# mnadareski/ZPAQSharp

Hardware: AMD Instinct MI355X
Metric: decompress MB/s (bit-exact) on 1 GiB multi-block stream (higher is better)
Workload: dtype u32; 1 GPU; BASELINE configs[1]: 256 x 4 MiB independent blocks per GPU, model l1 (1 component(s)), plaintext generator T; zpaq_model=l1, blocks_per_gpu=256, block_bytes=4194304, plaintext=T, parallelism=blocks x1, kernel_kind=2, blocks_in_flight=256

## Files before the change

zpaqsharp_amd/csrc/zh_cm.hip:

```cpp
#include <hip/hip_runtime.h>
#include <stddef.h>
#include <stdint.h>

#include "zh_core.h"
#include "zh_dev.h"
#include "zh_cm_fast.h"
#include "zh_model.h"

using namespace zhcore;
using namespace zhdev;

#pragma clang diagnostic ignored "-Wint-to-pointer-cast"

namespace {

constexpr uint32_t kNoWin = 0xFFFFFFFFu;
constexpr uint32_t kRing = 16;
enum : uint32_t { kMsgByte = 0, kMsgLeave = 2 };
enum : uint32_t { kCmdEnter = 1, kCmdExit = 3 };
constexpr uint32_t kSpinSection = 1u << 27;
constexpr uint64_t kSpinIdle = 1ull << 33;
#define ZH_E_HELPER (-24)

struct alignas(64) CmTabs {
  int16_t sh[16384];
  uint16_t sq[4096];
  int32_t dt[1024];
};
template <uint32_t NW>
struct alignas(64) CmBlkT {
  static constexpr uint32_t kNW = NW;
  uint32_t winB[NW][256];
  uint32_t winA[NW][16];
  uint16_t p16B[NW][256];
  uint16_t p16A[NW][16];
  alignas(64) uint32_t ring[kRing];
  uint32_t dummy[64];
  uint32_t aux[kRing][2];
  uint32_t tags[64];
  uint4 wsink[64];
  alignas(8) uint32_t mreq;
  uint32_t mold, mdone, mcfg;
  uint32_t t0, b_seq;
  uint32_t cmd_seq, cmd_code, cmd_ack;
  uint32_t limit, ob_word, ob_room;
  uint64_t table, ob_base, ob_cap, ob_len, ob_stored;
  uint32_t table_bytes;
  uint32_t pr[256];
  Vm pz;
  Sink sink;
};
template <uint32_t NW, uint32_t NP>
struct alignas(64) CmLdsT {
  CmTabs T;
  CmBlkT<NW> B[NP];
};
static_assert(sizeof(CmLdsT<64, 1>) <= 163840 && sizeof(CmLdsT<32, 2>) <= 163840, "LDS budget");
static_assert(offsetof(CmBlkT<64>, mold) == offsetof(CmBlkT<64>, mreq) + 4 && offsetof(CmBlkT<64>, mdone) == offsetof(CmBlkT<64>, mreq) + 8 && offsetof(CmBlkT<64>, mreq) % 8 == 0, "swap mailbox layout");

__device__ __forceinline__ uint32_t lds_ld(const uint32_t *p) {
  return __hip_atomic_load(p, __ATOMIC_RELAXED, __HIP_MEMORY_SCOPE_WORKGROUP);
}
__device__ __forceinline__ void lds_st(uint32_t *p, uint32_t v) {
  __hip_atomic_store(p, v, __ATOMIC_RELAXED, __HIP_MEMORY_SCOPE_WORKGROUP);
}
__device__ __forceinline__ void lds_put0(const uint32_t *where, uint32_t val) {
  const uint32_t addr = (uint32_t)(uintptr_t)where;
  asm volatile("s_mov_b64 exec, 1\n\tds_write_b32 %0, %1\n\ts_mov_b64 exec, -1" ::"v"(addr), "v"(val) : "memory");
}
__device__ __forceinline__ void lds_order() { asm volatile("" ::: "memory"); }
typedef __attribute__((address_space(3))) uint16_t *lds_u16_p;
typedef __attribute__((address_space(3))) uint32_t *lds_u32_p;
typedef __attribute__((address_space(3))) const uint64_t *lds_u64_p;
__device__ __forceinline__ uint32_t lds_u16(uint32_t off) { return *(lds_u16_p)off; }
__device__ __forceinline__ uint64_t lds_u64(uint32_t off) { return *(lds_u64_p)off; }
__device__ __forceinline__ uint32_t lds_off(const void *p) { return (uint32_t)(uintptr_t)p; }
__device__ __forceinline__ uint32_t p16b_pos(uint32_t q, uint32_t P) { return ((q & 3) << 6) | (P << 2) | (q >> 2); }
__device__ __forceinline__ uint32_t ring_tag(uint32_t u) { return u & 127u; }
static_assert(kRing == 16, "ring_tag");
__device__ __forceinline__ void wave_sync() { __builtin_amdgcn_fence(__ATOMIC_SEQ_CST, "workgroup"); }

__device__ __forceinline__ uint32_t p16_of(const CmTabs &T, uint32_t cm) {
  const uint32_t xv = cm >> 17;
  const int st = xv >= 16384 ? (int)T.sh[xv - 16384] : -(int)T.sh[16383 - xv];
  return (uint32_t)T.sq[st + 2048] * 2 + 1;
}

template <class BLK>
__device__ __forceinline__ void win_store(const BLK &S, uint32_t slot, uint32_t *table, uint32_t w, uint32_t lane) {
  uint4 *g = reinterpret_cast<uint4 *>(table + (uint64_t)w * 512);
// ... 143 lines not shown
    const uint32_t n = (r >> 23) & 255u;
    if (n == done) {
      const uint32_t c = uni(cfg_now);
      if (c == ~0u) break;
      if (++idle > 64) __builtin_amdgcn_s_sleep(2);
      if (idle > kSpinIdle) break;
      continue;
    }
    idle = 0;
    if (PROF) { asm volatile("s_memtime %0\n\ts_waitcnt lgkmcnt(0)" : "=s"(t_req)::"memory"); }
    const uint32_t c = uni(cfg_now);
    if (UNLIKELY(c != cfg)) {
      cfg = c;
      __builtin_amdgcn_fence(__ATOMIC_ACQUIRE, "workgroup");
      trs = __builtin_amdgcn_make_buffer_rsrc((void *)(L.arena + uni64(S.table)), 0, (int)uni(S.table_bytes), 0x00020000);
    }
    const uint32_t sl = r & 63u;
    const uint32_t neww = (r >> 22) & 1u ? uni(S.aux[0][0]) : (r >> 6) & 0xFFFFu;
    const uint32_t oldw = uni((uint32_t)(rq >> 32));
    const uint32_t aB = l_cB + sl * 1024u, aA = l_cA + sl * l_mA, aP = l_cP + sl * l_mP;
    const uint32_t so_new = neww * 2048u;
    const v4u nb = __builtin_amdgcn_raw_buffer_load_b128(trs, g_offB, so_new, 0);
    const v4u na = __builtin_amdgcn_raw_buffer_load_b128(trs, g_offA, so_new, 0);
    const v4u np = __builtin_amdgcn_raw_buffer_load_b128(trs, g_offP, so_new, 0);
    if (oldw != kNoWin) {
      const v4u vb = *(lds_v4_p)aB, va = *(lds_v4_p)aA, vp = *(lds_v4_p)aP;
      const uint32_t so_old = oldw * 2048u;
      __builtin_amdgcn_raw_buffer_store_b128(vb, trs, g_offB, so_old, 0);
      __builtin_amdgcn_raw_buffer_store_b128(va, trs, g_offA, so_old, 0);
      __builtin_amdgcn_raw_buffer_store_b128(vp, trs, g_offP, so_old, 0);
    }
    if (PROF) { asm volatile("s_memtime %0\n\ts_waitcnt lgkmcnt(0)" : "=s"(t_out)::"memory"); asm volatile("s_waitcnt vmcnt(3)" ::: "memory");
                asm volatile("s_memtime %0\n\ts_waitcnt lgkmcnt(0)" : "=s"(t_back)::"memory"); }
    *(lds_v4_p)aB = nb;
    *(lds_v4_p)aA = na;
    *(lds_v4_p)aP = np;
    lds_order();
    lds_put0(&S.mdone, n);
    done = n;
    if (PROF) { asm volatile("s_waitcnt lgkmcnt(0)\n\ts_memtime %0\n\ts_waitcnt lgkmcnt(0)" : "=s"(t_done)::"memory");
                c_a += t_out - t_req; c_b += t_back - t_out; c_c += t_done - t_back; ++n_sw; }
  }
  if (PROF && lane == 0 && L.debug) {
    atomicAdd((unsigned long long *)&L.debug[13], (unsigned long long)c_a);
    atomicAdd((unsigned long long *)&L.debug[14], (unsigned long long)c_b);
    atomicAdd((unsigned long long *)&L.debug[15], (unsigned long long)c_c);
    atomicAdd((unsigned long long *)&L.debug[9], (unsigned long long)n_sw);
  }
}

template <bool PROF, uint32_t NW, uint32_t NP>
__device__ __forceinline__ void decode_cm_body(const ZhLaunch &L, CmLdsT<NW, NP> &SS) {
  uint64_t prof[16] = {0, 0, 0, 0, 0, 0, 0, 0, 0, 0, 0, 0, 0, 0, 0, 0};
  uint64_t tprev = 0, t_exit = 0, t_pub = 0;
  bool was_miss = false;
  const uint32_t lane = threadIdx.x & 63, wid = threadIdx.x >> 6, pair = NP > 1 ? wid % NP : 0u, wave = NP > 1 ? wid / NP : wid;
  CmTabs &T = SS.T;
  CmBlkT<NW> &S = SS.B[pair];

  {
    const uint4 *s0 = reinterpret_cast<const uint4 *>(L.tables->stretch + 16384);
    uint4 *d0 = reinterpret_cast<uint4 *>(T.sh);
    for (uint32_t i = threadIdx.x; i < sizeof(T.sh) / 16; i += 192 * NP) d0[i] = s0[i];
    const uint4 *s1 = reinterpret_cast<const uint4 *>(L.tables->squash);
    uint4 *d1 = reinterpret_cast<uint4 *>(T.sq);
    for (uint32_t i = threadIdx.x; i < sizeof(T.sq) / 16; i += 192 * NP) d1[i] = s1[i];
    const uint4 *s2 = reinterpret_cast<const uint4 *>(L.tables->dt);
    uint4 *d2 = reinterpret_cast<uint4 *>(T.dt);
    for (uint32_t i = threadIdx.x; i < sizeof(T.dt) / 16; i += 192 * NP) d2[i] = s2[i];
    if (wave == 0 && lane == 0) { S.cmd_seq = 0; S.cmd_code = 0; S.cmd_ack = 0; S.t0 = 0; S.b_seq = 0; S.mreq = 0; S.mold = 0; S.mdone = 0; S.mcfg = 0; }
  }
  __syncthreads();
  if (wave == 1) { helper_wave<PROF>(L, T, S, lane); return; }
  if (wave == 2) { swap_wave<PROF>(L, S, lane); return; }
  uint32_t n_miss = 0, sec_cfg = 0;
  uint32_t cmd_seq = 0;

  const uint32_t l15 = lane & 15;
  const uint32_t lgrp = lane >> 4;
  const uint32_t ltt = 31 - __clz((int)(l15 | 1));
  const uint32_t lsh_vis = 4 - ltt, lsh_y = 3 - ltt;
  const uint32_t p_la = lds_off(&S.p16A[0][0]) + l15 * 2, p_lb = lds_off(&S.p16B[0][0]) + lgrp * 128 + l15 * 8;
  const uint32_t ring_addr = lds_off(&S.ring[0]), bseq_addr = lds_off(&S.b_seq), mreq_addr = lds_off(&S.mreq);
  const uint32_t dummy_addr = lds_off(&S.dummy[lane]), ring_step = lane == 0 ? 63u : 0u;

  uint8_t *slot_mem = L.arena + (uint64_t)(blockIdx.x * NP + pair) * L.arena_stride;

  for (;;) {
    uint32_t bi = 0;
    if (lane == 0) bi = atomicAdd(L.queue, 1u);
    bi = uni((uint32_t)__shfl((int)bi, 0));
    if (bi >= L.n_blocks) break;

    const ZhBlockDesc *bdp = &L.blocks[bi];
    const uint32_t model_i = uni(bdp->model);
    const uint32_t first_seg = uni(bdp->first_seg), n_seg = uni(bdp->n_seg);
    const uint64_t b_out_off = uni64(bdp->out_off), b_out_cap = uni64(bdp->out_cap);
    const ZhModel *M = &L.models[model_i];
    const ZhComp *cp = &M->comp[0];
    const uint32_t cm_mask = uni(cp->cm_mask);
    const uint32_t limit = (uint32_t)uni(cp->arg[1]) * 4;
    const uint64_t cm_off = uni64(cp->cm_off), cm_bytes = uni64(cp->cm_bytes);
    const uint32_t win_bfe = 9u | ((uint32_t)__builtin_popcount(cm_mask) - 9u) << 16;
    const uint32_t hshift = (uni(M->kind) >> 16) & 255;
    uint32_t *table = reinterpret_cast<uint32_t *>(slot_mem + cm_off);

    {
      const uint4 v = make_uint4(0x80000000u, 0x80000000u, 0x80000000u, 0x80000000u);
      uint4 *q = reinterpret_cast<uint4 *>(table);
      for (uint64_t i = lane; i < cm_bytes / 16; i += 64) q[i] = v;
      const uint32_t pv = p16_of(T, 0x80000000u), pp = pv | pv << 16;
      const uint4 ppat = make_uint4(pp, pp, pp, pp);
      const uint64_t nwin = cm_bytes / 2048;
      for (uint64_t i = lane; i < nwin * 34; i += 64) {
        const uint64_t w = i / 34, k = i % 34;
        q[w * 128 + (k < 32 ? 8 + k : 4 + (k - 32))] = ppat;
      }
      const uint64_t h_off = uni64(M->h_off), tail = uni64(M->arena_bytes) - h_off;
      uint4 *z = reinterpret_cast<uint4 *>(slot_mem + h_off);
      for (uint64_t i = lane; i < tail / 16; i += 64) z[i] = make_uint4(0, 0, 0, 0);
      for (uint32_t i = lane; i < 256; i += 64) S.pr[i] = 0;
    }
    wave_sync();

    uint32_t tag = kNoWin;
    uint32_t stale = 0;
    uint32_t lastuse = lane < NW ? 0u : ~0u;
    uint32_t thr = 1;
    uint32_t t = 0;
    uint32_t h0 = 0;

    int pp_state = 0, pp_hsize = 0;
    uint32_t pp_len = 0;
    Vm &pz = S.pz;
    pz.a = pz.b = pz.c = pz.d = pz.f = 0;
    pz.prog = nullptr; pz.len = 0;
    pz.m = slot_mem + uni64(M->pm_off); pz.mmask = (uint32_t)((1ull << uni(M->pm)) - 1);
    pz.h = reinterpret_cast<uint32_t *>(slot_mem + uni64(M->ph_off)); pz.hmask = (uint32_t)((1ull << uni(M->ph)) - 1);
    pz.r = S.pr;
    uint8_t *pzbuf = slot_mem + uni64(M->pz_off) + ZH_CODE_PAD;

    Dec d;
    d.low = 1; d.high = 0xFFFFFFFFu; d.curr = 0;

    OutBuf ob;
    ob.base = L.out + b_out_off; ob.cap = b_out_cap; ob.len = 0; ob.stored = 0; ob.word = 0; ob.park = 0;
    out_room(ob);
    Sink &sink = S.sink;
    sink.out = ob.base; sink.cap = ob.cap; sink.len = 0;

    wave_sync();
    InBuf in;
    in.stream = L.in; in.total = L.in_total; in.cbase = 0; in.k = 0; in.avail = 0; in.cur = 0;

    int failed = 0;
    for (uint32_t s = 0; s < n_seg; ++s) {
      const uint32_t si = first_seg + s;
      const uint64_t produced0 = pp_state == 5 ? uni64(sink.len) : ob.len;
      int status = 0;
      if (failed) {
        if (lane == 0) {
          ZhSegResult res;
          res.status = ZH_E_SKIPPED; res.pp_state = (uint32_t)pp_state; res.out_off = b_out_off + produced0; res.out_len = 0;
          res.in_used = 0;
          L.results[si] = res;
        }
// ... 68 lines not shown
          for (int i = 0; i < 4; ++i) {
            const uint32_t ps = rdlane(psel, lb + j2);
            ZH_DEC_STEP(d, ps, j2, bad, rn);
            if (UNLIKELY(rn)) { if (dec_renorm(d, in, lane) && !err) err = bad ? (uint32_t)-ZH_E_CORRUPT : (uint32_t)-ZH_E_EOF; }
          }
          if (UNLIKELY(err | bad)) { status = err ? -(int)err : ZH_E_CORRUPT; return -2; }
          ZH_STAMP(4);
          const uint32_t n2 = j2 & 15;
          c = (int)(n1 << 4 | n2);

          {
            const bool isb = lgrp == (ga & 3);
            const bool isa = lgrp == ((ga & 3) ^ 1);
            const uint32_t cmsel = kb == 0 ? cmb[0] : kb == 1 ? cmb[1] : kb == 2 ? cmb[2] : cmb[3];
            const uint32_t cm = isb ? cmsel : cma;
            const uint32_t nib = isb ? n2 : n1;
            const bool vis = (isa || isb) && l15 != 0 && l15 == ((16 | nib) >> lsh_vis);
            const uint32_t yy = (nib >> lsh_y) & 1;
            const uint32_t cnt = cm & 0x3ff;
            const int e = (int)(yy * 32767) - (int)(cm >> 17);
            const uint32_t nv = cm + (((uint32_t)e * (uint32_t)T.dt[cnt]) & 0xFFFFFC00u) + (cnt < limit);
            if (vis) { if (isb) wb[ib0 + 64 * kb] = nv; else wa[l15] = nv; }
          }
          ZH_STAMP(5);
          h0 = (uint32_t)c << hshift;
        }
        return (int)uni((uint32_t)c);
      };

      for (;;) {
        if (LIKELY(pp_state == 1)) {
          S.tags[lane] = stale;
          stale = 0;
          if (lane < kRing) S.ring[lane] = ((ring_tag(t) + 64) & 127) << 25;
          out_flush(ob, lane);
          if (lane == 0) {
            S.table = (uint64_t)(reinterpret_cast<uint8_t *>(table) - L.arena); S.limit = limit;
            S.table_bytes = (uint32_t)(cm_bytes > 0xFFFFF000ull ? 0xFFFFF000ull : cm_bytes);
            S.mcfg = ++sec_cfg;
            S.ob_base = (uint64_t)(ob.base - L.out); S.ob_cap = ob.cap; S.ob_len = ob.len; S.ob_stored = ob.stored;
            S.ob_word = ob.word; S.ob_room = ob.room;
            S.t0 = t; S.b_seq = t; S.cmd_code = kCmdEnter;
          }
          __builtin_amdgcn_fence(__ATOMIC_RELEASE, "workgroup");
          ++cmd_seq;
          lds_st(&S.cmd_seq, cmd_seq);
          bool helper_ok = true;
          {
            uint32_t sp = 0;
            while (lds_ld(&S.cmd_ack) != cmd_seq) { if (++sp > kSpinSection) { helper_ok = false; break; } }
            __builtin_amdgcn_fence(__ATOMIC_ACQUIRE, "workgroup");
          }
          if (!helper_ok) { status = ZH_E_HELPER; break; }
          uint32_t b_done = t;
          auto publish = [&](uint32_t m0) __attribute__((always_inline)) {
            lds_order();
            lds_put0(&S.ring[t & (kRing - 1)], ring_tag(t) << 25 | m0);
            ++t;
          };
          auto wait_done = [&](uint32_t upto) __attribute__((always_inline)) -> bool {
            uint32_t sp = 0;
            while ((int32_t)(b_done - upto) < 0) {
              b_done = uni(lds_ld(&S.b_seq));
              if (++sp > kSpinSection) return false;
            }
            lds_order();
            return true;
          };
          enum : uint32_t { kEvEos = 1, kEvCorrupt, kEvEof, kEvHelper };
          uint32_t ev = 0;
          uint32_t tq;
          for (;;) {
            {
              if (in.avail - in.k < 49 && in.avail == 256) in_seek(in, in_pos(in), lane);
              uint32_t code;
              d.low = uni(d.low); d.high = uni(d.high); d.curr = uni(d.curr); in.k = uni(in.k); in.avail = uni(in.avail);
              t = uni(t); h0 = uni(h0); b_done = uni(b_done); n_miss = uni(n_miss); thr = uni(thr);
              uint64_t f0 = 0, f1 = 0;
              const uint32_t t_in = t;
              if (PROF) { asm volatile("s_memtime %0\n\ts_waitcnt lgkmcnt(0)" : "=s"(f0)::"memory"); }
              if (LIKELY(d.curr - d.low <= d.high - d.low && t < 0x3e000000u)) {
                const uint32_t klim = uni(in.avail >= 48 ? in.avail - 48 : 0u);
                uint32_t vr = lane == 0 ? ring_addr + (t & (kRing - 1)) * 4u : dummy_addr;
                if (PROF) {
                  uint32_t sp_lo = 0, sp_hi = 0, nsp = 0;
                  ZH_CM_FAST_LOOP_PROF(d.low, d.high, d.curr, in.k, t, h0, b_done, lastuse, code, klim, uni(win_bfe), uni(hshift),
                                       vr, ring_step, bseq_addr, in.cur, tag, p_la, p_lb, thr, n_miss, mreq_addr, uni(kVictimBack<NW>), sp_lo, sp_hi, nsp);
                  prof[11] += (uint64_t)sp_hi << 32 | sp_lo; prof[12] += nsp;
                } else {
                ZH_CM_FAST_LOOP(d.low, d.high, d.curr, in.k, t, h0, b_done, lastuse, code, klim, uni(win_bfe), uni(hshift),
                                vr, ring_step, bseq_addr, in.cur, tag, p_la, p_lb, thr, n_miss, mreq_addr, uni(kVictimBack<NW>));
                }
              } else code = 0;
              if (PROF) { asm volatile("s_memtime %0\n\ts_waitcnt lgkmcnt(0)" : "=s"(f1)::"memory"); prof[2] += f1 - f0; prof[3] += t - t_in; t_exit = f1; }
              if (UNLIKELY(code)) { ev = kEvCorrupt; d.low = d.high = d.curr = 1; }
            }
            if (PROF) { asm volatile("s_memtime %0\n\ts_waitcnt lgkmcnt(0)" : "=s"(tprev)::"memory"); }
            if (UNLIKELY(d.curr == 0)) {
              uint32_t cu = 0;
              for (int i = 0; i < 4; ++i) cu = cu << 8 | (uint32_t)in_get(in, lane);
              d.curr = uni(cu);
            }
            tq = d.curr - d.low;
            if (UNLIKELY(tq - 1 >= d.high - d.low)) break;
            const uint32_t w = (h0 & cm_mask) >> 9;
            const uint64_t hit = __ballot(tag == w);
            if (UNLIKELY(hit == 0)) {
              thr = uni(thr);
              const uint32_t vs = uni(pick_victim<NW>(lastuse, t, thr));
              const uint32_t old = rdlane(tag, vs);
              tag = lane == vs ? w : tag;
              n_miss = uni(n_miss + 1);
              const uint32_t nn = n_miss & 255u;
              if (w >= 0x10000u && lane == 0) S.aux[0][0] = w;
              lds_st(&S.mold, old);
              lds_order();
              lds_put0(&S.mreq, nn << 23 | (w >= 0x10000u ? 1u << 22 : w << 6) | vs);
              lastuse = lane == vs ? (t > 13u ? t - 13u : 1u) : lastuse;
              if (PROF) { asm volatile("s_memtime %0\n\ts_waitcnt lgkmcnt(0)" : "=s"(t_pub)::"memory"); prof[8] += t_pub - t_exit; prof[10] += 1; }
              { uint32_t spn = 0; while (uni(lds_ld(&S.mdone)) != nn) { if (++spn > kSpinSection) { ev = kEvHelper; d.low = d.high = d.curr = 1; break; } } }
              lds_order();
              continue;
            }
            const uint32_t slot = (uint32_t)__builtin_ctzll(hit);
            uint32_t bad = 0, err = 0, helper_lost = 0;
            {
              uint32_t spn = 0;
              while (UNLIKELY(uni(lds_ld(&S.mdone)) != (n_miss & 255u))) { if (++spn > kSpinSection) { helper_lost = 1; break; } }
              lds_order();
            }
            d.low += 1;
            if (UNLIKELY((d.high ^ d.low) < 0x1000000u)) {
              if (dec_renorm_chk(d, in, lane, bad)) err = kEvEof;
            }
            ZH_STAMP(0);
            {
              const uint32_t since = t - rdlane(lastuse, slot);
              const uint32_t back = since < kRing - 3 ? since : kRing - 3;
              if (UNLIKELY(t - b_done > back)) { if (!wait_done(t - back)) helper_lost = 1; }
            }
            ZH_STAMP(1);
            const uint32_t pa = (uint32_t)lds_u16(p_la + slot * 32) << 16;
            const uint64_t pb = lds_u64(p_lb + slot * 512);
            uint32_t j = 1;
#pragma unroll
            for (int tt = 0; tt < 4; ++tt) {
              const uint32_t ps = rdlane(pa, j);
              uint32_t xr;
              ZH_DEC_STEP_LITE(d, ps, j, xr);
              if (UNLIKELY(xr < 0x1000000u)) {
                const uint32_t was = bad;
                if (dec_renorm_chk(d, in, lane, bad) && !err) err = was ? kEvCorrupt : kEvEof;
              }
            }
            const uint32_t ga = uni(j & 15), lb = (ga & 3) * 16;
            const uint32_t psel = (uint32_t)(pb >> ((ga >> 2) * 16)) << 16;
            uint32_t j2 = 1;
#pragma unroll
            for (int tt = 0; tt < 4; ++tt) {
              const uint32_t ps = rdlane(psel, lb + j2);
              uint32_t xr;
              ZH_DEC_STEP_LITE(d, ps, j2, xr);
              if (UNLIKELY(xr < 0x1000000u)) {
                uint32_t later = 0;
                const uint32_t was = bad;
                if (dec_renorm_chk(d, in, lane, tt == 3 ? later : bad) && !err) err = was ? kEvCorrupt : kEvEof;
              }
            }
            ZH_STAMP(4);
            if (LIKELY((err | bad | helper_lost) == 0)) {
              const uint32_t cc = (j << 4) + j2 - 272;
              publish(kMsgByte << 23 | cc << 15 | slot);
              lastuse = lane == slot ? t : lastuse;
              h0 = cc << hshift;
            } else {
// ... 102 lines not shown
```

zpaqsharp_amd/csrc/zh_cm_fast.h:

```cpp
#pragma once

#define ZH_FAST_STEP_(PV, IDX, N, ADDC, SHADOW)                       \
  "v_readlane_b32 s94, " PV ", " IDX "\n\t"                           \
  SHADOW                                                              \
  "s_sub_u32 s84, %[high], %[low]\n\t"                                \
  "s_mul_hi_u32 s86, s84, s94\n\t"                                    \
  "s_add_u32 s87, %[low], s86\n\t"                                    \
  "s_add_u32 s88, s87, 1\n\t"                                         \
  "s_cmp_le_u32 %[curr], s87\n\t"                                     \
  "s_cselect_b32 %[high], s87, %[high]\n\t"                           \
  "s_cselect_b32 %[low], %[low], s88\n\t"                             \
  ADDC "\n\t"                                                         \
  "s_xor_b32 s84, %[high], %[low]\n\t"                                \
  "s_cmp_lt_u32 s84, %[c24]\n\t"                                      \
  "s_cbranch_scc1 .Lzh_rn" #N "_%=\n"                                 \
  ".Lzh_bk" #N "_%=:\n\t"
#define ZH_FAST_ADDC_IDX(J) "s_addc_u32 " J ", " J ", " J "\n\ts_add_u32 s80, s89, " J
#define ZH_FAST_ADDC1_IDX(J) "s_addc_u32 " J ", 1, 1\n\ts_add_u32 s80, s89, " J

#ifndef ZH_L1_COLD_ALIGN
#define ZH_L1_COLD_ALIGN 1
#endif
#if ZH_L1_COLD_ALIGN
#define ZH_FAST_COLD_ALIGN ".p2align 5\n"
#else
#define ZH_FAST_COLD_ALIGN ""
#endif
#define ZH_FAST_SHIFT_IN(N)                                           \
  ".Lzh_rl" #N "_%=:\n\t"                                             \
  "s_lshl_b32 %[high], %[high], 8\n\t"                                \
  "s_or_b32 %[high], %[high], 0xff\n\t"                               \
  "s_lshl_b32 %[low], %[low], 8\n\t"                                  \
  "s_max_u32 %[low], %[low], 1\n\t"                                   \
  "s_lshr_b32 s84, %[k], 2\n\t"                                       \
  "v_readlane_b32 s85, %[cur], s84\n\t"                               \
  "s_lshl_b32 s84, %[k], 3\n\t"                                       \
  "s_lshr_b32 s85, s85, s84\n\t"                                      \
  "s_and_b32 s85, s85, 0xff\n\t"                                      \
  "s_lshl_b32 %[curr], %[curr], 8\n\t"                                \
  "s_or_b32 %[curr], %[curr], s85\n\t"                                \
  "s_add_u32 %[k], %[k], 1\n\t"                                       \
  "s_xor_b32 s84, %[high], %[low]\n\t"                                \
  "s_cmp_lt_u32 s84, 0x1000000\n\t"                                   \
  "s_cbranch_scc1 .Lzh_rl" #N "_%=\n\t"
#define ZH_FAST_RENORM(N)                                             \
  ZH_FAST_COLD_ALIGN                                                  \
  ".Lzh_rn" #N "_%=:\n\t"                                             \
  ZH_FAST_SHIFT_IN(N)                                                 \
  ZH_FAST_CHK                                                         \
  "s_branch .Lzh_bk" #N "_%=\n\t"
#define ZH_FAST_RENORM_LAST(N, S)                                     \
  ZH_FAST_COLD_ALIGN                                                  \
  ".Lzh_rn" #N "_%=:\n\t"                                             \
  ZH_FAST_SHIFT_IN(N)                                                 \
  ZH_FAST_CHK8(S)                                                     \
  "s_branch .Lzh_bk" #N "_%=\n\t"

#define ZH_FAST_CHK                                                   \
  "s_cmp_lt_u32 %[curr], %[low]\n\t"                                  \
  "s_cbranch_scc1 .Lzh_corrupt_%=\n\t"                                \
  "s_cmp_gt_u32 %[curr], %[high]\n\t"                                 \
  "s_cbranch_scc1 .Lzh_corrupt_%=\n\t"

#define ZH_FAST_CHK8(S)                                               \
  "s_cmp_lt_u32 %[curr], %[low]\n\t"                                  \
  "s_cbranch_scc1 .Lzh_oor" #S "_%=\n\t"                              \
  "s_cmp_gt_u32 %[curr], %[high]\n\t"                                 \
  "s_cbranch_scc1 .Lzh_oor" #S "_%=\n\t"

#define ZH_FAST_READ_BSEQ "ds_read_b32 v245, %[bsa]\n\t"
#define ZH_FAST_SHADOW1 "v_readfirstlane_b32 %[bdone], v245\n\tv_mov_b32_e32 v243, s82\n\tv_add_u32_e32 v238, -12, v241\n\t"
#define ZH_FAST_SHADOW2 "v_add_u32_e32 v252, 1, v241\n\tv_cndmask_b32_e32 %[lu], %[lu], v252, vcc\n\tv_nop\n\t"
#define ZH_FAST_SHADOW3 "v_lshl_or_b32 v243, v241, 25, v243\n\tv_nop\n\t"
#define ZH_FAST_SHADOW4 "v_nop\n\tv_nop\n\tv_nop\n\t"
#define ZH_FAST_SHADOW5 "v_add_u32_e32 v251, 4, %[vr]\n\tv_nop\n\t"
#define ZH_FAST_SHADOW6 "v_bfi_b32 v251, %[vm], v251, %[vr]\n\t"
#define ZH_FAST_SHADOW7 "v_sub_u32_e32 v239, %[k], v240\n\tv_or_b32_e32 v239, v237, v239\n\t"
#define ZH_FAST_SHADOW8 "v_max3_i32 v242, v238, %[lu], v239\n\tv_add_u32_e32 v241, 1, v241\n\t"
#define ZH_FAST_LAGV "v_add_u32_e32 v244, -13, v241\n\tv_sub_u32_e32 v239, %[k], v240\n\tv_or_b32_e32 v239, v237, v239\n\tv_max3_i32 v242, v244, %[lu], v239\n\t"
#define ZH_FAST_ENTRY "v_mov_b32_e32 v241, %[t]\n\tv_mov_b32_e32 v240, %[klim]\n\tv_mov_b32_e32 v237, 0x40000000\n\t"
#define ZH_FAST_T "v_readfirstlane_b32 %[t], v241\n\t"
#define ZH_FAST_EPILOGUE                                              \
  "s_lshl4_add_u32 s92, s90, s91\n\t"                                 \
  "s_addk_i32 s92, 0xfef0\n\t"                                        \
  "v_lshl_or_b32 v250, s92, 15, v243\n\t"                             \
  "ds_write_b32 %[vr], v250\n\t"                                      \
  "v_mov_b32_e32 %[vr], v251\n\t"                                     \
  "s_lshl_b32 %[h0], s92, %[hs]\n\t"
#define ZH_FAST_LOOKUP(S)                                             \
  "s_bfe_u32 s81, %[h0], %[bfe]\n\t"                                  \
  "v_cmp_eq_u32_e32 vcc, s81, %[tag]\n\t"                             \
  "v_cmp_gt_i32_e64 s[76:77], v242, %[bdone]\n\t"                     \
  "s_cbranch_vccz .Lzh_miss_%=\n\t"                                   \
  "s_ff1_i32_b64 s82, vcc\n\t"                                        \
  "s_and_b64 s[76:77], s[76:77], vcc\n\t"                             \
  "s_cbranch_scc1 .Lzh_fresh" #S "_%=\n"
#define ZH_FAST_FRESH_IN ZH_FAST_T "s_cmp_ge_u32 %[k], %[klim]\n\ts_cbranch_scc1 .Lzh_slow_%=\n\tv_readlane_b32 s83, %[lu], s82\n\ts_sub_u32 s83, %[t], s83\n\ts_min_u32 s83, s83, 13\n\t"
#define ZH_FAST_BITS(N1, N2, N3, N4, N5, N6, N7, N8)                  \
  ZH_FAST_STEP_("v249", "1", N1, "s_addc_u32 s90, 1, 1", ZH_FAST_SHADOW1)\
  ZH_FAST_STEP_("v249", "s90", N2, "s_addc_u32 s90, s90, s90", ZH_FAST_SHADOW2)\
  ZH_FAST_STEP_("v249", "s90", N3, "s_addc_u32 s90, s90, s90", ZH_FAST_SHADOW3)\
  ZH_FAST_STEP_("v249", "s90", N4, "s_addc_u32 s90, s90, s90", ZH_FAST_SHADOW4)    \
  "s_and_b32 s89, s90, 3\n\t"                                         \
  "s_lshl_b32 s89, s89, 4\n\t"                                        \
  "s_lshl_b32 s83, s90, 2\n\t"                                        \
  "s_and_b32 s83, s83, 48\n\t"                                        \
  "s_add_u32 s80, s89, 1\n\t"                                         \
  "v_lshrrev_b64 v[250:251], s83, v[250:251]\n\t"                     \
  "v_lshlrev_b32_e32 v250, 16, v250\n\t"                              \
  ZH_FAST_STEP_("v250", "s80", N5, ZH_FAST_ADDC1_IDX("s91"), ZH_FAST_SHADOW5)      \
  ZH_FAST_STEP_("v250", "s80", N6, ZH_FAST_ADDC_IDX("s91"), ZH_FAST_SHADOW6)\
  ZH_FAST_STEP_("v250", "s80", N7, ZH_FAST_ADDC_IDX("s91"), ZH_FAST_SHADOW7)\
  ZH_FAST_STEP_("v250", "s80", N8, "s_addc_u32 s91, s91, s91", ZH_FAST_SHADOW8)
#define ZH_CM_FAST_BYTE(S, E, N1, N2, N3, N4, N5, N6, N7, N8, H0, H1, H2, H3) \
  H0                                                                  \
  ZH_FAST_LOOKUP(S)                                                   \
  ".Lzh_ok" #S "_%=:\n\t"                                             \
  H1                                                                  \
   \
   \
  "v_lshl_add_u32 v252, s82, 5, %[la]\n\t"                            \
  "v_lshl_add_u32 v250, s82, 9, %[lb]\n\t"                            \
  "ds_read_u16_d16_hi v249, v252\n\t"                                 \
  "ds_read_b64 v[250:251], v250\n\t"                                  \
  ZH_FAST_READ_BSEQ                                                   \
   \
   \
  "s_cmp_le_u32 %[curr], %[low]\n\t"                                  \
  "s_cbranch_scc1 .Lzh_slow_%=\n\t"                                   \
  "s_add_u32 %[low], %[low], 1\n\t"                                   \
   \
  "s_and_b32 s84, %[low], %[c24m]\n\t"                                \
  "s_cbranch_scc0 .Lzh_e0" #S "_%=\n"                                 \
  ".Lzh_bk" #E "_%=:\n\t"                                             \
  "s_waitcnt lgkmcnt(0)\n\t"                                          \
  H2                                                                  \
  ZH_FAST_BITS(N1, N2, N3, N4, N5, N6, N7, N8)                        \
  H3                                                                  \
  ZH_FAST_EPILOGUE
#define ZH_FAST_OK_DIRECT(S) ".Lzh_ok" #S "_%="
#define ZH_FAST_OK_STAMPED(S) ".Lzh_okp" #S "_%="
#define ZH_CM_FAST_COLD(S, E, N1, N2, N3, N4, N5, N6, N7, N8, SPIN_IN, SPIN_OK) \
   \
  ZH_FAST_COLD_ALIGN                                                  \
  ".Lzh_fresh" #S "_%=:\n\t"                                          \
  ZH_FAST_FRESH_IN                                                    \
  SPIN_IN                                                             \
  "s_mov_b32 s80, 48\n"                                               \
  ".Lzh_spin" #S "_%=:\n\t"                                           \
  "ds_read_b32 v252, %[bsa]\n\t"                                      \
  "s_waitcnt lgkmcnt(0)\n\t"                                          \
  "v_readfirstlane_b32 %[bdone], v252\n\t"                            \
  "s_sub_u32 s89, %[t], %[bdone]\n\t"                                 \
  "s_cmp_gt_u32 s89, s83\n\t"                                         \
  "s_cbranch_scc0 " SPIN_OK(S) "\n\t"                                 \
  "s_sub_u32 s80, s80, 1\n\t"                                         \
  "s_cmp_lg_u32 s80, 0\n\t"                                           \
  "s_cbranch_scc1 .Lzh_spin" #S "_%=\n\t"                             \
  "s_branch .Lzh_slow_%=\n\t"                                         \
  ZH_FAST_COLD_ALIGN                                                  \
  ".Lzh_e0" #S "_%=:\n\t"                                             \
  "s_xor_b32 s84, %[high], %[low]\n\t"                                \
  "s_cmp_lt_u32 s84, %[c24]\n\t"                                      \
  "s_cbranch_scc0 .Lzh_bk" #E "_%=\n\t"                               \
  "s_branch .Lzh_rn" #E "_%=\n\t"                                     \
  ZH_FAST_RENORM(E)                                                   \
  ZH_FAST_RENORM(N1)                                                  \
  ZH_FAST_RENORM(N2)                                                  \
  ZH_FAST_RENORM(N3)                                                  \
  ZH_FAST_RENORM(N4)                                                  \
  ZH_FAST_RENORM(N5)                                                  \
  ZH_FAST_RENORM(N6)                                                  \
  ZH_FAST_RENORM(N7)                                                  \
  ZH_FAST_RENORM_LAST(N8, S)                                          \
  ".Lzh_oor" #S "_%=:\n\t"                                            \
  ZH_FAST_EPILOGUE                                                    \
  "s_branch .Lzh_slow_%=\n"

#ifndef ZH_L1_PAD
#define ZH_L1_PAD 4
#endif
#define ZH_STR_(x) #x
#define ZH_STR(x) ZH_STR_(x)
#define ZH_FAST_PAD ".fill " ZH_STR(ZH_L1_PAD) ", 4, 0xbf800000\n"
#define ZH_FAST_MISS_BLOCK                                            \
   \
  ZH_FAST_COLD_ALIGN                                                  \
  ".Lzh_miss_%=:\n\t"                                                 \
  ZH_FAST_T                                                           \
  "s_cmp_ge_u32 s81, 0x10000\n\t"                                     \
  "s_cbranch_scc1 .Lzh_slow_%=\n\t"                                   \
  "v_cmp_gt_u32_e32 vcc, %[thr], %[lu]\n\t"                           \
  "s_cbranch_vccnz .Lzh_mvic_%=\n\t"                                  \
   \
  "s_sub_u32 %[thr], %[t], %[kb]\n\t"                                 \
  "s_max_i32 %[thr], %[thr], 1\n\t"                                   \
  "v_cmp_gt_u32_e32 vcc, %[thr], %[lu]\n\t"                           \
  "s_cbranch_vccz .Lzh_slow_%=\n"                                     \
  ".Lzh_mvic_%=:\n\t"                                                 \
  "s_ff1_i32_b64 s82, vcc\n\t"                                        \
  "s_mov_b32 s84, m0\n\t"                                             \
  "s_mov_b32 m0, s82\n\t"                                             \
  "s_add_u32 %[nm], %[nm], 1\n\t"                                     \
  "s_and_b32 s85, %[nm], 0xff\n\t"                                    \
  "s_lshl_b32 s80, s85, 23\n\t"                                       \
  "s_lshl_b32 s86, s81, 6\n\t"                                        \
  "s_or_b32 s80, s80, s86\n\t"                                        \
  "s_or_b32 s80, s80, s82\n\t"                                        \
  "v_readlane_b32 s83, %[tag], m0\n\t"                                \
  "v_writelane_b32 %[tag], s81, m0\n\t"                               \
  "v_mov_b32_e32 v250, s83\n\t"                                       \
  "ds_write_b32 %[mqa], v250 offset:4\n\t"                            \
  "v_mov_b32_e32 v250, s80\n\t"                                       \
  "ds_write_b32 %[mqa], v250\n\t"                                     \
  "s_sub_u32 s87, %[t], 13\n\t"                                       \
  "s_max_i32 s87, s87, 1\n\t"                                         \
  "v_writelane_b32 %[lu], s87, m0\n\t"                                \
  ZH_FAST_LAGV                                                        \
  "s_mov_b32 m0, s84\n\t"                                             \
  "s_mov_b32 s80, 0x4000\n"                                           \
  ".Lzh_mspin_%=:\n\t"                                                \
  "ds_read_b32 v252, %[mqa] offset:8\n\t"                             \
  "s_waitcnt lgkmcnt(0)\n\t"                                          \
  "v_readfirstlane_b32 s86, v252\n\t"                                 \
  "s_cmp_eq_u32 s86, s85\n\t"                                         \
  "s_cbranch_scc1 .Lzh_byte_%=\n\t"                                   \
  "s_sub_u32 s80, s80, 1\n\t"                                         \
  "s_cmp_lg_u32 s80, 0\n\t"                                           \
  "s_cbranch_scc1 .Lzh_mspin_%=\n\t"                                  \
  "s_branch .Lzh_slow_%=\n"
#define ZH_CM_FAST_LOOP(low_, high_, curr_, k_, t_, h0_, bdone_, lu_, code_, klim_, bfe_, hs_, vr_, vm_, bsa_, cur_, tag_, la_, lb_, thr_, nm_, mqa_, kb_) \
  asm volatile(                                                       \
  "v_mov_b32_e32 v249, 0\n\t"                                         \
  ZH_FAST_ENTRY                                                       \
  ZH_FAST_LAGV                                                        \
  "s_branch .Lzh_byte_%=\n\t"    \
  ".p2align 8\n"                                                      \
  ZH_FAST_PAD                                                         \
  ".Lzh_byte_%=:\n\t"                                                 \
  ZH_CM_FAST_BYTE(a, 0, 1, 2, 3, 4, 5, 6, 7, 8, "", "", "", "")       \
  ZH_CM_FAST_BYTE(b, 10, 11, 12, 13, 14, 15, 16, 17, 18, "", "", "", "") \
  "s_branch .Lzh_byte_%=\n"                                           \
                                           \
  ZH_CM_FAST_COLD(a, 0, 1, 2, 3, 4, 5, 6, 7, 8, "", ZH_FAST_OK_DIRECT)               \
  ZH_CM_FAST_COLD(b, 10, 11, 12, 13, 14, 15, 16, 17, 18, "", ZH_FAST_OK_DIRECT)      \
  ZH_FAST_MISS_BLOCK                                                  \
  ".Lzh_corrupt_%=:\n\t"                                              \
  "s_mov_b32 %[code], 1\n\t"                                          \
  "s_branch .Lzh_end_%=\n"                                            \
  ".Lzh_slow_%=:\n\t"                                                 \
  "s_waitcnt lgkmcnt(0)\n\t"                                          \
  "s_mov_b32 %[code], 0\n"                                            \
  ".Lzh_end_%=:\n\t"                                                  \
  ZH_FAST_T                                                           \
  : [low] "+s"(low_), [high] "+s"(high_), [curr] "+s"(curr_), [k] "+s"(k_), [t] "+s"(t_), [h0] "+s"(h0_), \
    [bdone] "+s"(bdone_), [lu] "+v"(lu_), [vr] "+v"(vr_), [tag] "+v"(tag_), [nm] "+s"(nm_), [thr] "+s"(thr_), [code] "=s"(code_)          \
  : [klim] "s"(klim_), [bfe] "s"(bfe_), [hs] "s"(hs_), [vm] "v"(vm_), [bsa] "v"(bsa_),             \
    [cur] "v"(cur_), [la] "v"(la_), [lb] "v"(lb_), [mqa] "v"(mqa_), [kb] "s"(kb_), [c24] "s"(0x1000000u), [c24m] "s"(0xffffffu)                      \
  : "memory", "scc", "vcc", "s80", "s81", "s82", "s83", "s84", "s85", "s86", "s87", "s88", "s89", "s90",   \
    "s91", "s92", "s94", "v249", "v250", "v251", "v252", "v245", "s76", "s77", "v237", "v238", "v239", "v240", "v241", "v242", "v243", "v244")
#ifndef ZH_L1_STAGE
#define ZH_L1_STAGE 0
#endif
#define ZH_STG_A "s_memtime s[96:97]\n\t"
#define ZH_STG_B "s_memtime s[98:99]\n\t"
#define ZH_STG_ACC "s_sub_u32 s98, s98, s96\n\ts_subb_u32 s99, s99, s97\n\ts_add_u32 s100, s100, s98\n\ts_addc_u32 s101, s101, s99\n\t"
#if ZH_L1_STAGE == 1
#define ZH_STG_H0 ZH_STG_A
#define ZH_STG_H1 ZH_STG_B
#define ZH_STG_H2 ZH_STG_ACC
#define ZH_STG_H3 ""
#elif ZH_L1_STAGE == 2
#define ZH_STG_H0 ""
#define ZH_STG_H1 ZH_STG_A
#define ZH_STG_H2 ZH_STG_B
#define ZH_STG_H3 "s_waitcnt lgkmcnt(0)\n\t" ZH_STG_ACC
#elif ZH_L1_STAGE == 3
#define ZH_STG_H0 ""
#define ZH_STG_H1 ""
#define ZH_STG_H2 ZH_STG_ACC ZH_STG_A
#define ZH_STG_H3 ZH_STG_B
#elif ZH_L1_STAGE == 4
#define ZH_STG_H0 ZH_STG_B
#define ZH_STG_H1 ""
#define ZH_STG_H2 ZH_STG_ACC
#define ZH_STG_H3 ZH_STG_A
#else
#define ZH_STG_H0 ""
#define ZH_STG_H1 ""
#define ZH_STG_H2 ""
#define ZH_STG_H3 ""
#endif
#define ZH_FAST_SPIN_IN "s_memtime s[96:97]\n\t"
#define ZH_FAST_SPIN_OK(S) ".Lzh_okp" #S "_%=:\n\ts_memtime s[98:99]\n\ts_waitcnt lgkmcnt(0)\n\ts_sub_u32 s98, s98, s96\n\ts_subb_u32 s99, s99, s97\n\ts_add_u32 s100, s100, s98\n\ts_addc_u32 s101, s101, s99\n\ts_add_u32 %[nspin], %[nspin], 1\n\ts_branch .Lzh_ok" #S "_%=\n\t"
#if ZH_L1_STAGE
#define ZH_PROF_SPIN_IN ""
#define ZH_PROF_SPIN_OKL ZH_FAST_OK_DIRECT
#define ZH_PROF_SPIN_OKB(S) ""
#else
#define ZH_PROF_SPIN_IN ZH_FAST_SPIN_IN
#define ZH_PROF_SPIN_OKL ZH_FAST_OK_STAMPED
#define ZH_PROF_SPIN_OKB(S) ZH_FAST_SPIN_OK(S)
#endif
#define ZH_CM_FAST_LOOP_PROF(low_, high_, curr_, k_, t_, h0_, bdone_, lu_, code_, klim_, bfe_, hs_, vr_, vm_, bsa_, cur_, tag_, la_, lb_, thr_, nm_, mqa_, kb_, spin_lo_, spin_hi_, nspin_) \
  asm volatile(                                                       \
  "v_mov_b32_e32 v249, 0\n\t"                                         \
  ZH_FAST_ENTRY                                                       \
  ZH_FAST_LAGV                                                        \
  "s_mov_b32 s100, 0\n\t"                                             \
  "s_mov_b32 s101, 0\n\t"                                             \
  "s_memtime s[96:97]\n\t"                                            \
  "s_waitcnt lgkmcnt(0)\n\t"                                          \
  "s_mov_b32 s98, s96\n\t"                                            \
  "s_mov_b32 s99, s97\n\t"                                            \
  "s_branch .Lzh_byte_%=\n\t"                                         \
  ".p2align 8\n"                                                      \
  ZH_FAST_PAD                                                         \
  ".Lzh_byte_%=:\n\t"                                                 \
  ZH_CM_FAST_BYTE(a, 0, 1, 2, 3, 4, 5, 6, 7, 8, ZH_STG_H0, ZH_STG_H1, ZH_STG_H2, ZH_STG_H3)       \
  ZH_CM_FAST_BYTE(b, 10, 11, 12, 13, 14, 15, 16, 17, 18, ZH_STG_H0, ZH_STG_H1, ZH_STG_H2, ZH_STG_H3) \
  "s_branch .Lzh_byte_%=\n"                                           \
  ZH_CM_FAST_COLD(a, 0, 1, 2, 3, 4, 5, 6, 7, 8, ZH_PROF_SPIN_IN, ZH_PROF_SPIN_OKL)              \
  ZH_CM_FAST_COLD(b, 10, 11, 12, 13, 14, 15, 16, 17, 18, ZH_PROF_SPIN_IN, ZH_PROF_SPIN_OKL)     \
  ZH_PROF_SPIN_OKB(a)                                                 \
  ZH_PROF_SPIN_OKB(b)                                                 \
  ZH_FAST_MISS_BLOCK                                                  \
  ".Lzh_corrupt_%=:\n\t"                                              \
  "s_mov_b32 %[code], 1\n\t"                                          \
  "s_branch .Lzh_end_%=\n"                                            \
  ".Lzh_slow_%=:\n\t"                                                 \
  "s_waitcnt lgkmcnt(0)\n\t"                                          \
  "s_mov_b32 %[code], 0\n"                                            \
  ".Lzh_end_%=:\n\t"                                                  \
  ZH_FAST_T                                                           \
  "s_mov_b32 %[splo], s100\n\t"                                       \
  "s_mov_b32 %[sphi], s101\n\t"                                       \
  : [low] "+s"(low_), [high] "+s"(high_), [curr] "+s"(curr_), [k] "+s"(k_), [t] "+s"(t_), [h0] "+s"(h0_), \
    [bdone] "+s"(bdone_), [lu] "+v"(lu_), [vr] "+v"(vr_), [tag] "+v"(tag_), [nm] "+s"(nm_), [thr] "+s"(thr_), [code] "=s"(code_), [splo] "=s"(spin_lo_), [sphi] "=s"(spin_hi_), [nspin] "+s"(nspin_) \
  : [klim] "s"(klim_), [bfe] "s"(bfe_), [hs] "s"(hs_), [vm] "v"(vm_), [bsa] "v"(bsa_),             \
    [cur] "v"(cur_), [la] "v"(la_), [lb] "v"(lb_), [mqa] "v"(mqa_), [kb] "s"(kb_), [c24] "s"(0x1000000u), [c24m] "s"(0xffffffu)                      \
  : "memory", "scc", "vcc", "s80", "s81", "s82", "s83", "s84", "s85", "s86", "s87", "s88", "s89", "s90",   \
    "s91", "s92", "s94", "s96", "s97", "s98", "s99", "s100", "s101", "v249", "v250", "v251", "v252", "v245", "s76", "s77", "v237", "v238", "v239", "v240", "v241", "v242", "v243", "v244")
```

Baseline: 666.9 MB/s.

## Refill compressed input window inside fast CM loop with prefetched global loads

Instead of leaving the inline-asm fast decode loop for the slow path whenever the input window runs low, the loop now prefetches the next 192-byte input chunk per lane with a global_load into a spare VGPR. When the window is exhausted it swaps in that chunk, rebases k, advances the chunk base and issues the next prefetch, then continues decoding. The aim is to avoid frequent slow-path exits and window reseeks on the hot path. In exchange it adds a vmcnt wait at loop exit, two more clobbered VGPRs, and extra bookkeeping of the remaining input length, with some risk around the end of the stream.

```diff
diff --git a/zpaqsharp_amd/csrc/zh_cm.hip b/zpaqsharp_amd/csrc/zh_cm.hip
--- a/zpaqsharp_amd/csrc/zh_cm.hip
+++ b/zpaqsharp_amd/csrc/zh_cm.hip
@@ -6,6 +6,10 @@
 #include "zh_dev.h"
 #include "zh_cm_fast.h"
 #include "zh_model.h"
+
+#ifndef ZH_L1_REFILL
+#define ZH_L1_REFILL 1
+#endif
 
 using namespace zhcore;
 using namespace zhdev;
@@ -315,6 +319,7 @@
   const uint32_t lsh_vis = 4 - ltt, lsh_y = 3 - ltt;
   const uint32_t p_la = lds_off(&S.p16A[0][0]) + l15 * 2, p_lb = lds_off(&S.p16B[0][0]) + lgrp * 128 + l15 * 8;
   const uint32_t ring_addr = lds_off(&S.ring[0]), bseq_addr = lds_off(&S.b_seq), mreq_addr = lds_off(&S.mreq);
+  const uint32_t lane4 = lane * 4u;
   const uint32_t dummy_addr = lds_off(&S.dummy[lane]), ring_step = lane == 0 ? 63u : 0u;
 
   uint8_t *slot_mem = L.arena + (uint64_t)(blockIdx.x * NP + pair) * L.arena_stride;
@@ -549,15 +554,21 @@
               if (LIKELY(d.curr - d.low <= d.high - d.low && t < 0x3e000000u)) {
                 const uint32_t klim = uni(in.avail >= 48 ? in.avail - 48 : 0u);
                 uint32_t vr = lane == 0 ? ring_addr + (t & (kRing - 1)) * 4u : dummy_addr;
+                const uint64_t in_left = uni64(in.total > in.cbase ? in.total - in.cbase : 0);
+                uint32_t room = ZH_L1_REFILL && in_left >= 448 ? (uint32_t)(in_left - 448 < (1ull << 30) ? in_left - 448 : 1ull << 30) + 192u : 0u;
+                uint32_t adv = 0;
+                room = uni(room);
+                const uint64_t chunk_at = uni64((uint64_t)(uintptr_t)in.stream + in.cbase);
                 if (PROF) {
                   uint32_t sp_lo = 0, sp_hi = 0, nsp = 0;
                   ZH_CM_FAST_LOOP_PROF(d.low, d.high, d.curr, in.k, t, h0, b_done, lastuse, code, klim, uni(win_bfe), uni(hshift),
-                                       vr, ring_step, bseq_addr, in.cur, tag, p_la, p_lb, thr, n_miss, mreq_addr, uni(kVictimBack<NW>), sp_lo, sp_hi, nsp);
+                                       vr, ring_step, bseq_addr, in.cur, tag, p_la, p_lb, thr, n_miss, mreq_addr, uni(kVictimBack<NW>), room, adv, chunk_at, lane4, sp_lo, sp_hi, nsp);
                   prof[11] += (uint64_t)sp_hi << 32 | sp_lo; prof[12] += nsp;
                 } else {
                 ZH_CM_FAST_LOOP(d.low, d.high, d.curr, in.k, t, h0, b_done, lastuse, code, klim, uni(win_bfe), uni(hshift),
-                                vr, ring_step, bseq_addr, in.cur, tag, p_la, p_lb, thr, n_miss, mreq_addr, uni(kVictimBack<NW>));
+                                vr, ring_step, bseq_addr, in.cur, tag, p_la, p_lb, thr, n_miss, mreq_addr, uni(kVictimBack<NW>), room, adv, chunk_at, lane4);
                 }
+                in.cbase += uni(adv);
               } else code = 0;
               if (PROF) { asm volatile("s_memtime %0\n\ts_waitcnt lgkmcnt(0)" : "=s"(f1)::"memory"); prof[2] += f1 - f0; prof[3] += t - t_in; t_exit = f1; }
               if (UNLIKELY(code)) { ev = kEvCorrupt; d.low = d.high = d.curr = 1; }
diff --git a/zpaqsharp_amd/csrc/zh_cm_fast.h b/zpaqsharp_amd/csrc/zh_cm_fast.h
--- a/zpaqsharp_amd/csrc/zh_cm_fast.h
+++ b/zpaqsharp_amd/csrc/zh_cm_fast.h
@@ -95,7 +95,7 @@
   "s_ff1_i32_b64 s82, vcc\n\t"                                        \
   "s_and_b64 s[76:77], s[76:77], vcc\n\t"                             \
   "s_cbranch_scc1 .Lzh_fresh" #S "_%=\n"
-#define ZH_FAST_FRESH_IN ZH_FAST_T "s_cmp_ge_u32 %[k], %[klim]\n\ts_cbranch_scc1 .Lzh_slow_%=\n\tv_readlane_b32 s83, %[lu], s82\n\ts_sub_u32 s83, %[t], s83\n\ts_min_u32 s83, s83, 13\n\t"
+#define ZH_FAST_FRESH_IN ZH_FAST_T "s_cmp_ge_u32 %[k], %[klim]\n\ts_cbranch_scc1 .Lzh_refill_%=\n\tv_readlane_b32 s83, %[lu], s82\n\ts_sub_u32 s83, %[t], s83\n\ts_min_u32 s83, s83, 13\n\t"
 #define ZH_FAST_BITS(N1, N2, N3, N4, N5, N6, N7, N8)                  \
   ZH_FAST_STEP_("v249", "1", N1, "s_addc_u32 s90, 1, 1", ZH_FAST_SHADOW1)\
   ZH_FAST_STEP_("v249", "s90", N2, "s_addc_u32 s90, s90, s90", ZH_FAST_SHADOW2)\
@@ -229,11 +229,32 @@
   "s_cmp_lg_u32 s80, 0\n\t"                                           \
   "s_cbranch_scc1 .Lzh_mspin_%=\n\t"                                  \
   "s_branch .Lzh_slow_%=\n"
-#define ZH_CM_FAST_LOOP(low_, high_, curr_, k_, t_, h0_, bdone_, lu_, code_, klim_, bfe_, hs_, vr_, vm_, bsa_, cur_, tag_, la_, lb_, thr_, nm_, mqa_, kb_) \
+#define ZH_FAST_NXT_LOAD(L)                                           \
+  "s_cmp_lt_u32 %[room], 0xc0\n\t"                                    \
+  "s_cbranch_scc1 " L "\n\t"                                          \
+  "global_load_dword v246, v247, %[sb]\n"                             \
+  L ":\n\t"
+#define ZH_FAST_PRIME "v_add_u32_e32 v247, 0xc0, %[l4]\n\t" ZH_FAST_NXT_LOAD(".Lzh_prm_%=")
+#define ZH_FAST_REFILL_BLOCK                                          \
+  ZH_FAST_COLD_ALIGN                                                  \
+  ".Lzh_refill_%=:\n\t"                                               \
+  "s_cmp_lt_u32 %[room], 0xc0\n\t"                                    \
+  "s_cbranch_scc1 .Lzh_slow_%=\n\t"                                   \
+  "s_waitcnt vmcnt(0)\n\t"                                            \
+  "v_mov_b32_e32 %[cur], v246\n\t"                                    \
+  "v_add_u32_e32 v247, 0xc0, v247\n\t"                                \
+  "s_sub_u32 %[k], %[k], 0xc0\n\t"                                    \
+  "s_add_u32 %[adv], %[adv], 0xc0\n\t"                                \
+  "s_sub_u32 %[room], %[room], 0xc0\n\t"                              \
+  ZH_FAST_NXT_LOAD(".Lzh_rfd_%=")                                     \
+  ZH_FAST_LAGV                                                        \
+  "s_branch .Lzh_byte_%=\n\t"
+#define ZH_CM_FAST_LOOP(low_, high_, curr_, k_, t_, h0_, bdone_, lu_, code_, klim_, bfe_, hs_, vr_, vm_, bsa_, cur_, tag_, la_, lb_, thr_, nm_, mqa_, kb_, room_, adv_, sb_, l4_) \
   asm volatile(                                                       \
   "v_mov_b32_e32 v249, 0\n\t"                                         \
   ZH_FAST_ENTRY                                                       \
   ZH_FAST_LAGV                                                        \
+  ZH_FAST_PRIME                                                       \
   "s_branch .Lzh_byte_%=\n\t"    \
   ".p2align 8\n"                                                      \
   ZH_FAST_PAD                                                         \
@@ -245,6 +266,7 @@
   ZH_CM_FAST_COLD(a, 0, 1, 2, 3, 4, 5, 6, 7, 8, "", ZH_FAST_OK_DIRECT)               \
   ZH_CM_FAST_COLD(b, 10, 11, 12, 13, 14, 15, 16, 17, 18, "", ZH_FAST_OK_DIRECT)      \
   ZH_FAST_MISS_BLOCK                                                  \
+  ZH_FAST_REFILL_BLOCK                                                \
   ".Lzh_corrupt_%=:\n\t"                                              \
   "s_mov_b32 %[code], 1\n\t"                                          \
   "s_branch .Lzh_end_%=\n"                                            \
@@ -252,13 +274,14 @@
   "s_waitcnt lgkmcnt(0)\n\t"                                          \
   "s_mov_b32 %[code], 0\n"                                            \
   ".Lzh_end_%=:\n\t"                                                  \
+  "s_waitcnt vmcnt(0)\n\t"      \
   ZH_FAST_T                                                           \
   : [low] "+s"(low_), [high] "+s"(high_), [curr] "+s"(curr_), [k] "+s"(k_), [t] "+s"(t_), [h0] "+s"(h0_), \
-    [bdone] "+s"(bdone_), [lu] "+v"(lu_), [vr] "+v"(vr_), [tag] "+v"(tag_), [nm] "+s"(nm_), [thr] "+s"(thr_), [code] "=s"(code_)          \
+    [bdone] "+s"(bdone_), [lu] "+v"(lu_), [vr] "+v"(vr_), [tag] "+v"(tag_), [cur] "+v"(cur_), [room] "+s"(room_), [adv] "+s"(adv_), [nm] "+s"(nm_), [thr] "+s"(thr_), [code] "=s"(code_)          \
   : [klim] "s"(klim_), [bfe] "s"(bfe_), [hs] "s"(hs_), [vm] "v"(vm_), [bsa] "v"(bsa_),             \
-    [cur] "v"(cur_), [la] "v"(la_), [lb] "v"(lb_), [mqa] "v"(mqa_), [kb] "s"(kb_), [c24] "s"(0x1000000u), [c24m] "s"(0xffffffu)                      \
+    [sb] "s"(sb_), [l4] "v"(l4_), [la] "v"(la_), [lb] "v"(lb_), [mqa] "v"(mqa_), [kb] "s"(kb_), [c24] "s"(0x1000000u), [c24m] "s"(0xffffffu)                      \
   : "memory", "scc", "vcc", "s80", "s81", "s82", "s83", "s84", "s85", "s86", "s87", "s88", "s89", "s90",   \
-    "s91", "s92", "s94", "v249", "v250", "v251", "v252", "v245", "s76", "s77", "v237", "v238", "v239", "v240", "v241", "v242", "v243", "v244")
+    "s91", "s92", "s94", "v249", "v250", "v251", "v252", "v245", "s76", "s77", "v237", "v238", "v239", "v240", "v241", "v242", "v243", "v244", "v246", "v247")
 #ifndef ZH_L1_STAGE
 #define ZH_L1_STAGE 0
 #endif
@@ -302,11 +325,12 @@
 #define ZH_PROF_SPIN_OKL ZH_FAST_OK_STAMPED
 #define ZH_PROF_SPIN_OKB(S) ZH_FAST_SPIN_OK(S)
 #endif
-#define ZH_CM_FAST_LOOP_PROF(low_, high_, curr_, k_, t_, h0_, bdone_, lu_, code_, klim_, bfe_, hs_, vr_, vm_, bsa_, cur_, tag_, la_, lb_, thr_, nm_, mqa_, kb_, spin_lo_, spin_hi_, nspin_) \
+#define ZH_CM_FAST_LOOP_PROF(low_, high_, curr_, k_, t_, h0_, bdone_, lu_, code_, klim_, bfe_, hs_, vr_, vm_, bsa_, cur_, tag_, la_, lb_, thr_, nm_, mqa_, kb_, room_, adv_, sb_, l4_, spin_lo_, spin_hi_, nspin_) \
   asm volatile(                                                       \
   "v_mov_b32_e32 v249, 0\n\t"                                         \
   ZH_FAST_ENTRY                                                       \
   ZH_FAST_LAGV                                                        \
+  ZH_FAST_PRIME                                                       \
   "s_mov_b32 s100, 0\n\t"                                             \
   "s_mov_b32 s101, 0\n\t"                                             \
   "s_memtime s[96:97]\n\t"                                            \
@@ -325,6 +349,7 @@
   ZH_PROF_SPIN_OKB(a)                                                 \
   ZH_PROF_SPIN_OKB(b)                                                 \
   ZH_FAST_MISS_BLOCK                                                  \
+  ZH_FAST_REFILL_BLOCK                                                \
   ".Lzh_corrupt_%=:\n\t"                                              \
   "s_mov_b32 %[code], 1\n\t"                                          \
   "s_branch .Lzh_end_%=\n"                                            \
@@ -332,12 +357,13 @@
   "s_waitcnt lgkmcnt(0)\n\t"                                          \
   "s_mov_b32 %[code], 0\n"                                            \
   ".Lzh_end_%=:\n\t"                                                  \
+  "s_waitcnt vmcnt(0)\n\t"      \
   ZH_FAST_T                                                           \
   "s_mov_b32 %[splo], s100\n\t"                                       \
   "s_mov_b32 %[sphi], s101\n\t"                                       \
   : [low] "+s"(low_), [high] "+s"(high_), [curr] "+s"(curr_), [k] "+s"(k_), [t] "+s"(t_), [h0] "+s"(h0_), \
-    [bdone] "+s"(bdone_), [lu] "+v"(lu_), [vr] "+v"(vr_), [tag] "+v"(tag_), [nm] "+s"(nm_), [thr] "+s"(thr_), [code] "=s"(code_), [splo] "=s"(spin_lo_), [sphi] "=s"(spin_hi_), [nspin] "+s"(nspin_) \
+    [bdone] "+s"(bdone_), [lu] "+v"(lu_), [vr] "+v"(vr_), [tag] "+v"(tag_), [cur] "+v"(cur_), [room] "+s"(room_), [adv] "+s"(adv_), [nm] "+s"(nm_), [thr] "+s"(thr_), [code] "=s"(code_), [splo] "=s"(spin_lo_), [sphi] "=s"(spin_hi_), [nspin] "+s"(nspin_) \
   : [klim] "s"(klim_), [bfe] "s"(bfe_), [hs] "s"(hs_), [vm] "v"(vm_), [bsa] "v"(bsa_),             \
-    [cur] "v"(cur_), [la] "v"(la_), [lb] "v"(lb_), [mqa] "v"(mqa_), [kb] "s"(kb_), [c24] "s"(0x1000000u), [c24m] "s"(0xffffffu)                      \
+    [sb] "s"(sb_), [l4] "v"(l4_), [la] "v"(la_), [lb] "v"(lb_), [mqa] "v"(mqa_), [kb] "s"(kb_), [c24] "s"(0x1000000u), [c24m] "s"(0xffffffu)                      \
   : "memory", "scc", "vcc", "s80", "s81", "s82", "s83", "s84", "s85", "s86", "s87", "s88", "s89", "s90",   \
-    "s91", "s92", "s94", "s96", "s97", "s98", "s99", "s100", "s101", "v249", "v250", "v251", "v252", "v245", "s76", "s77", "v237", "v238", "v239", "v240", "v241", "v242", "v243", "v244")
+    "s91", "s92", "s94", "s96", "s97", "s98", "s99", "s100", "s101", "v249", "v250", "v251", "v252", "v245", "s76", "s77", "v237", "v238", "v239", "v240", "v241", "v242", "v243", "v244", "v246", "v247")
```

Result: no change. 670.2 MB/s, median of 6 (+0.5%).
